# mikekatz04/Eryn

Measured on AMD Instinct MI355X. Metric: walker-steps/sec (ntemps x nwalkers x iters/s), Gaussian logL, higher is better.
Workload: dtype f64; 1 GPU; config 2: ntemps=16, nwalkers=4096, ndim=32 dense-covariance Gaussian, box prior +-50, StretchMove(a=2)+adaptive PT, Philox RNG; ntemps=16, nwalkers=4096, ndim=32, parallelism=single GPU

## Files before the change

### eryn_amd/csrc/hens_kernels.h

```cpp
#pragma once
#include <hip/hip_runtime.h>
#include <stdint.h>
#include <type_traits>

namespace hens {

constexpr int TILE = 64;
constexpr unsigned FLAG_NONFINITE_X = 1u;
constexpr unsigned FLAG_NAN_LOGL = 2u;

constexpr unsigned FLAG_PIPE_TIMEOUT = 4u;

enum { LIKE_DENSE = 0, LIKE_DIAG = 1, LIKE_ROSEN = 2, LIKE_HOST = 3 };
enum { MODE_STRETCH = 0, MODE_EVAL = 1, MODE_MH = 2 };

struct u4 { uint32_t x, y, z, w; };

__device__ __forceinline__ u4 philox4x32_10(u4 c, uint32_t k0, uint32_t k1) {
#pragma unroll
    for (int r = 0; r < 10; ++r) {
        const uint32_t hi0 = __umulhi(0xD2511F53u, c.x), lo0 = 0xD2511F53u * c.x;
        const uint32_t hi1 = __umulhi(0xCD9E8D57u, c.z), lo1 = 0xCD9E8D57u * c.z;
        c = u4{hi1 ^ c.y ^ k0, lo1, hi0 ^ c.w ^ k1, lo0};
        k0 += 0x9E3779B9u;
// ... 2188 lines not shown
            A.dbg_uacc[base + q] = sd.ua;
        }
    }
}

inline __global__ void k_plan_keys(const PlanArgs A, int nb) {
    const int g = blockIdx.x * blockDim.x + threadIdx.x;
    if (g >= nb * A.Tl) return;
    const int ib = g / A.Tl, job = g - ib * A.Tl;
    const uint32_t rung = (uint32_t)(A.rung_begin + job);
    const PrpKey K = prp_key(A.seed, A.iter0 + (uint64_t)ib, PURPOSE_PTPERM, rung);
    uint32_t* dst = A.keys + ((size_t)ib * A.T + rung) * 8;
#pragma unroll
    for (int r = 0; r < 8; ++r) dst[r] = K.k[r];
}

inline __global__ __launch_bounds__(256) void k_plan_draws(const PlanArgs A) {
    const int ib = blockIdx.y / A.Tl, job = blockIdx.y - ib * A.Tl;
    const uint32_t rung = (uint32_t)(A.rung_begin + job);
    const uint64_t it = A.iter0 + (uint64_t)ib;
    const int W = A.W, hb = A.cb >> 1, hb_shift = __ffs(hb) - 1, N0 = W >> 1;
    const int q = blockIdx.x * 256 + threadIdx.x;
    if (q >= W) return;
    const uint4* kp = reinterpret_cast<const uint4*>(A.keys + ((size_t)ib * A.T + rung) * 8);
    const uint4 ka = kp[0], kb = kp[1];
    const uint32_t key[8] = {ka.x, ka.y, ka.z, ka.w, kb.x, kb.y, kb.z, kb.w};
    const size_t base = ((size_t)ib * A.Tl + job) * W;
    const bool s0 = q < N0;
    const int p = s0 ? q : q - N0;
    const PlaceDraw pd = stretch_draws_at(A.seed, it, rung, q, key, W, A.idx_bits, hb_shift);
    const DrawRec rc = draw_values(pd.own, pd.cw, pd.uz, pd.ua, A.a, A.D);
    const int blk = p >> hb_shift, ml = p & (hb - 1);
    const size_t ri = ((size_t)ib * (W / A.cb) + blk) * TILE + (size_t)rung * hb + ml;
    if (A.rec1) {
        if (s0) {
            A.rec1[ri] = rc;
        } else {
            A.rec[ri] = rc;
            const PlaceDraw p1 = stretch_draws_at(A.seed, it, rung, pd.r, key, W, A.idx_bits, hb_shift);
            A.rec3[ri] = draw_values(p1.own, p1.cw, p1.uz, p1.ua, A.a, A.D);
        }
        return;
    }
    A.dr.own[base + q] = rc.own;
    if (s0 || !(A.rec && A.rec_only)) {
        A.dr.cw[base + q] = rc.cw;
        A.dr.zz[base + q] = rc.zz;
        A.dr.fac[base + q] = rc.fac;
        A.dr.lu[base + q] = rc.lu;
    }
    if (A.rec && !s0) A.rec[ri] = rc;
    if (A.dbg_uzz) {
        A.dbg_uzz[base + q] = pd.uz;
        A.dbg_uacc[base + q] = pd.ua;
    }
}

inline __global__ void k_pt_invert(const int64_t* __restrict__ iperm, int32_t* __restrict__ inv, int npairs, int W) {
    const int64_t n = (int64_t)npairs * W;
    for (int64_t i = blockIdx.x * (int64_t)blockDim.x + threadIdx.x; i < n; i += (int64_t)gridDim.x * blockDim.x) {
        const int j = (int)(i / W);
        inv[(size_t)j * W + iperm[i]] = (int32_t)(i - (int64_t)j * W);
    }
}

inline __global__ void k_pt_chain(const int64_t* __restrict__ iperm, const int64_t* __restrict__ i1perm,
                           const int32_t* __restrict__ inv, const double* __restrict__ u_swap,
                           int32_t* __restrict__ colslot, int32_t* __restrict__ colk,
                           double* __restrict__ colu, int T, int W) {
    const int c = blockIdx.x * blockDim.x + threadIdx.x;
    if (c >= W) return;
    int k = c;
    for (int j = 0; j < T - 1; ++j) {
        const int i = T - 1 - j;
        if (j == 0) colslot[(size_t)i * W + c] = (int32_t)iperm[k];
        const int b = (int)i1perm[(size_t)j * W + k];
        colslot[(size_t)(i - 1) * W + c] = b;
        colk[(size_t)j * W + c] = k;
        colu[(size_t)j * W + c] = u_swap[(size_t)j * W + k];
        if (j + 1 < T - 1) k = inv[(size_t)(j + 1) * W + b];
    }
}

struct PtArgs {
    const double* Lfull;
    const double* P;
    const int32_t* loc;
    double* Lnew;
    double* Pnew;
    int32_t* locnew;
    const WalkerRec* wrec;
    WalkerRec* wrecnew;
    const double* betas;
    const int32_t* colslot;
    const double* colu;
    uint8_t* selcol;
    int32_t* srcfull;
    uint32_t* swap_part;
    uint64_t iter;
    uint64_t seed;
    unsigned long long* trace;
    int32_t T, W, Tl, rung_begin, idx_bits;
    int32_t acc_rows;
};

constexpr int PT_COLS = 16;
constexpr int PT_THREADS = 256;
__host__ __device__ inline int pt_threads(int T) { const int ne = (T * 16 + 63) & ~63; return ne < 256 ? 256 : (ne > 1024 ? 1024 : ne); }

__host__ __device__ inline size_t pt_lds_layout(int T) { return (size_t)T * PT_COLS * (8 + 8 + 8 + 4 + 4) + (size_t)T * 8 + (size_t)PT_COLS * ((T + 31) / 32) * 4; }

template <bool PHILOX>
__global__ __launch_bounds__(1024) void k_pt_cascade(const PtArgs A) {
    extern __shared__ __attribute__((aligned(16))) char smem_raw[];
    const int T = A.T, W = A.W;
    const size_t NE = (size_t)T * PT_COLS;
    double* Lc = reinterpret_cast<double*>(smem_raw);
    double* lu = Lc + NE;
    double* Pc = lu + NE;
    double* sbeta = Pc + NE;
    int32_t* locc = reinterpret_cast<int32_t*>(sbeta + T);
    int32_t* scol = locc + NE;
    uint32_t* smask = reinterpret_cast<uint32_t*>(scol + NE);
    const int MW = (T + 31) / 32;
    const int tid = threadIdx.x;
    const int NTH = blockDim.x;
    const int c0 = blockIdx.x * PT_COLS;
    const uint64_t it = A.iter;
#define PT_TRACE(i) do { if (A.trace && tid == 0) A.trace[(size_t)blockIdx.x * 8 + (i)] = trace_stamp(); } while (0)
    PT_TRACE(0);

    for (int t = tid; t < T; t += NTH) sbeta[t] = A.betas[t];
    constexpr int PT_KEEP = 2;
    uint32_t acc_keep[PT_KEEP] = {0u, 0u};
    for (int e = tid, k = 0; e < (int)NE; e += NTH, ++k) {
        const int t = e / PT_COLS, cc = e - t * PT_COLS, c = c0 + cc;
        if (c < W) {
            const int slot = PHILOX ? pt_slot(A.seed, it, t, T, c, A.idx_bits, W) : A.colslot[(size_t)t * W + c];
            scol[e] = slot;
            const int tl = t - A.rung_begin;
            if (A.wrec) {
                const WalkerRec wr = A.wrec[(size_t)t * W + slot];
                Lc[e] = wr.L; Pc[e] = wr.P; locc[e] = wr.loc;
                if (k == 0) acc_keep[0] = wr.acc;
                if (k == 1) acc_keep[1] = wr.acc;
            } else {
                Lc[e] = A.Lfull[(size_t)t * W + slot];
                if (tl >= 0 && tl < A.Tl) {
                    Pc[e] = A.P[(size_t)tl * W + slot];
                    locc[e] = A.loc[(size_t)tl * W + slot];
                } else {
                    locc[e] = -1;
                }
            }
            if (t < T - 1) {
                const double u = PHILOX ? pt_uniform(A.seed, it, t, W, c) : A.colu[(size_t)t * W + c];
                lu[e] = log(u);
            }
        }
    }
    PT_TRACE(1);
    PT_TRACE(2);
    __syncthreads();
    PT_TRACE(3);

    auto walk = [&](auto tt) {
        constexpr int TT = decltype(tt)::value;
        const int Tn = TT ? TT : T;
        const int cc = tid;
        double cL = Lc[(size_t)(Tn - 1) * PT_COLS + cc];
        uint32_t m = 0;
#pragma unroll
        for (int i0 = Tn - 1; i0 >= 1; i0 -= 8) {
            double Lb[8], lv[8], db[8];
#pragma unroll
            for (int q = 0; q < 8; ++q) {
                const int i = (i0 - q >= 1) ? i0 - q : 1;
                Lb[q] = Lc[(size_t)(i - 1) * PT_COLS + cc];
                lv[q] = lu[(size_t)(Tn - 1 - i) * PT_COLS + cc];
                db[q] = sbeta[i - 1] - sbeta[i];
            }
#pragma unroll
            for (int q = 0; q < 8; ++q) {
                const int i = i0 - q;
                if (i >= 1) {
                    const double pacc = db[q] * (cL - Lb[q]);
                    const bool sw = pacc > lv[q];
                    m |= sw ? (1u << (i & 31)) : 0u;
                    cL = sw ? cL : Lb[q];
                    if ((i & 31) == 0 || i == 1) {
                        smask[cc * MW + (i >> 5)] = m;
                        m = 0;
                    }
                }
            }
        }
    };
    if (tid < PT_COLS && c0 + tid < W) {
        if (T == 8) walk(std::integral_constant<int, 8>{});
        else if (T == 16) walk(std::integral_constant<int, 16>{});
        else if (T == 32) walk(std::integral_constant<int, 32>{});
        else walk(std::integral_constant<int, 0>{});
    }
    PT_TRACE(4);
    __syncthreads();
    PT_TRACE(5);

    auto bit = [&](int cc, int i) -> bool { return (i >= 1 && i < T) && ((smask[cc * MW + (i >> 5)] >> (i & 31)) & 1u); };
    for (int e = tid, k = 0; e < (int)NE; e += NTH, ++k) {
        const int t = e / PT_COLS, cc = e - t * PT_COLS, c = c0 + cc;
        if (c >= W) continue;
        int st;
        bool sel_out;
        if (MW == 1) {
            const uint32_t mw = smask[cc];
            sel_out = (mw >> ((T - 1 - t) & 31)) & 1u;
            if ((mw >> t) & 1u) st = t - 1;
            else st = t + __builtin_ctz(~(mw >> 1 >> t));
        } else {
            sel_out = bit(cc, T - 1 - t);
            if (bit(cc, t)) {
                st = t - 1;
            } else {
                st = t;
                while (bit(cc, st + 1)) ++st;
            }
        }
        if (t < T - 1 && A.selcol) A.selcol[(size_t)t * W + c] = sel_out ? 1 : 0;
        const int se = st * PT_COLS + cc;
        const int dslot = scol[e];
        if (A.srcfull) A.srcfull[(size_t)t * W + dslot] = st * W + scol[se];
        const int tl = t - A.rung_begin;
        if (tl < 0 || tl >= A.Tl) continue;
        const size_t di = (size_t)tl * W + dslot;
        if (A.wrecnew) {
            const uint32_t acc_own = (k < PT_KEEP && A.rung_begin == 0) ? (k == 0 ? acc_keep[0] : acc_keep[1]) : A.wrec[di].acc;
            A.wrecnew[di] = make_wrec(Lc[se], Pc[se], locc[se], acc_own);
            A.locnew[di] = locc[se];
            continue;
        }
        A.Lnew[di] = Lc[se];
        A.locnew[di] = locc[se];
        if (locc[se] >= 0) A.Pnew[di] = Pc[se];
    }
    for (int i = 1 + tid; i < T; i += NTH) {
        unsigned n = 0;
        for (int cc = 0; cc < PT_COLS && c0 + cc < W; ++cc) n += bit(cc, i) ? 1u : 0u;
        if (A.acc_rows) { if (n) atomicAdd(&A.swap_part[(size_t)(blockIdx.x & (A.acc_rows - 1)) * (T - 1) + (i - 1)], n); }
        else A.swap_part[(size_t)blockIdx.x * (T - 1) + (i - 1)] = n;
    }
    PT_TRACE(6);
#undef PT_TRACE
}

constexpr int SWAP_ACC_ROWS_MAX = 64;
__host__ __device__ inline int acc_row_groups(int T) {
    int p2 = 1;
    while (p2 < T - 1) p2 <<= 1;
    const int g = p2 >= 64 ? 1 : 64 / p2;
    return g > SWAP_ACC_ROWS_MAX / 8 ? SWAP_ACC_ROWS_MAX / 8 : g;
}

struct FusedArgs {
    double* pool;
    const WalkerRec* wrec;
    WalkerRec* wrecnew;
    const int32_t* loc;
    int32_t* locnew;
    const double* betas;
    const uint32_t* keys;
    const uint32_t* keys_next;
    uint32_t* accepted;
    uint32_t* swap_acc;
    const double* lo; const double* hi; const double* mu; const double* prec; const double* prec_sym;
    const double* period;
    unsigned* flags;
    unsigned long long* trace;
    double logp_in, fill, rosen_a, rosen_b;
    double a;
    uint64_t iter, seed;
    int32_t T, W, idx_bits, cb, cb_shift, ndim_active;
    int32_t acc_rows;
    int32_t norel;
    int32_t Tl, rung_begin;
    int32_t cbl, cbl_shift;
    int64_t guest_delta;
    int32_t* ghome;
    char* box; char* box_hot; char* box_cold;
    const double* pool_cold;
    unsigned long long* stats;
    long long budget;
    uint32_t sweep;
    int32_t par, nranks, rank;
    int32_t sys_rows;
    int32_t no_move;
};

__host__ __device__ constexpr size_t fused_lds_base(int D, int NW, bool pipe = false) {
    return ((size_t)TILE * (D + 2) + (size_t)NW * TILE + 5 * TILE + 3 * 2 * TILE + 64 + (pipe ? 2 * TILE : 0)) * 8 +
           (2 * 2 * TILE + 5 * TILE + 64 + (pipe ? 3 * TILE : 0)) * 4;
}
__host__ __device__ inline size_t fused_lds_bytes(int D, int NW, int like, bool pipe = false) { return fused_lds_base(D, NW, pipe) + mf_lds_extra(D, like); }

template <int DT, int LIKE, int NW, bool PER = false, bool SHORT = false, bool PIPE = false, bool COL = false>
__global__ __launch_bounds__(NW * 64) void k_split1_pt(const FusedArgs A) {
    static_assert(DT == 8 || DT == 16 || DT == 32 || DT == 64 || DT == 128, "power-of-two row width");
    static_assert(!(PIPE && SHORT), "pipeline ranks: full tiles");
    static_assert(!(COL && (PER || SHORT)), "column-ordered records: full tiles");
    extern __shared__ __attribute__((aligned(16))) char smem_raw[];
    constexpr bool CEN = like_centred(LIKE, DT);
    constexpr int D = DT, RS = DT + 2, NT = NW * 64, LPR = DT / 2, RPP = NT / LPR, NPASS = (TILE + RPP - 1) / RPP;
    constexpr int NE = 2 * TILE;
    constexpr int NEX = PIPE ? NE + TILE : NE;
    static_assert(NT >= 2 * NE, "one thread per slot + one per cascade uniform");
    constexpr bool WIDE = NT >= 2 * NE + 64;
    double* qtile = reinterpret_cast<double*>(smem_raw);
    double* s_part = qtile + TILE * RS;
    double* s_zz = s_part + NW * TILE;
    double* s_fac = s_zz + TILE;
    double* s_lu = s_fac + TILE;
    double* s_Lold = s_lu + TILE;
    double* s_Pold = s_Lold + TILE;
    int2* s_own = reinterpret_cast<int2*>(s_Lold);
    double* Lc = s_Pold + TILE;
    double* Pc = Lc + NEX;
    double* lupt = Pc + NEX;
    double* sbeta = lupt + NE;
    int32_t* locc = reinterpret_cast<int32_t*>(sbeta + 64);
    int32_t* scol = locc + NEX;
    int32_t* s_rs = scol + NE;
    int32_t* s_rc = s_rs + TILE;
    int32_t* s_dst = s_rc + TILE;
    int32_t* s_flag = s_dst + TILE;
    int32_t* s_el = s_flag + TILE;
    uint32_t* smask = reinterpret_cast<uint32_t*>(s_el + TILE);
    int32_t* s_src = reinterpret_cast<int32_t*>(smask + 64);
    int32_t* s_yrow = s_src + TILE;
    double* s_mu = reinterpret_cast<double*>(smem_raw + fused_lds_base(DT, NW, PIPE));

    const int tid = threadIdx.x;
    const int lane = tid & 63;
    const int wv = __builtin_amdgcn_readfirstlane(tid >> 6);
    if constexpr (like_mf<DT, LIKE, NW>()) {
        if (tid >= NW * 64 - DT / 2) *reinterpret_cast<double2*>(s_mu + 2 * (tid - (NW * 64 - DT / 2))) = *reinterpret_cast<const double2*>(A.mu + 2 * (tid - (NW * 64 - DT / 2)));
    }
    MfRegs mfr = like_prefetch<DT == 32 ? DT : 0, LIKE, NW>(lane, wv, A.prec_sym);
    const int TG = A.T;
    const int T = PIPE ? A.Tl : A.T;
    const int W = A.W, CB = PIPE ? A.cbl : A.cb, CS = PIPE ? A.cbl_shift : A.cb_shift;
    const int R0 = PIPE ? A.rung_begin : 0;
    const bool has_top = PIPE && R0 + T < TG, has_bot = PIPE && R0 > 0;
    const int TE = T + (has_top ? 1 : 0);
    const int c0 = blockIdx.x * CB;
    const int MW = (TE + 31) >> 5;
    const int NEr = SHORT ? (T << CS) : 2 * TILE, NM = SHORT ? (NEr >> 1) : TILE;
#define FUSED_TRACE(i) do { if (A.trace && tid == 0) A.trace[(size_t)blockIdx.x * 8 + (i)] = trace_stamp(); } while (0)
    FUSED_TRACE(0);
#ifdef HENS_DEV_BUILD
    if (HENS_CUT_F == 9) return;
#endif
#ifdef HENS_DEV_BUILD
    if (HENS_CUT_F == 8) {
        const long long t0 = wall_clock64();
        while (wall_clock64() - t0 < 600) __builtin_amdgcn_s_sleep(4);
        return;
    }
#endif

    WalkerRec wr_n{};
    bool stays = false;
    int slot_n = 0;
    int32_t home_n = 0;
    const int HS = A.cb_shift - 1, HB = 1 << HS;
    const int HW = CB >> 1;
    const bool nomove = PIPE && A.no_move != 0;
    constexpr int CWW = WIDE ? 5 : 2, FLW = WIDE ? 6 : 3;
    auto mover_of = [&](int t, int cc) -> int {
        if (PIPE) return (t << (CS - 1)) + ((cc >> (HS + 1)) << HS) + (cc & (HB - 1));
        return (t << (CS - 1)) + cc - HB;
    };
    if (wv == 0) s_flag[lane] = 0;
    if (tid < NEr) {
        const int e = tid, t = e >> CS, cc = e & (CB - 1), c = c0 + cc;
        if (COL) {
            wr_n = A.wrec[(size_t)t * W + c];
        } else {
            const uint4* kp = reinterpret_cast<const uint4*>(A.keys) + (size_t)(R0 + t) * 2;
            const uint4 ka = kp[0], kb = kp[1];
            const uint32_t key[8] = {ka.x, ka.y, ka.z, ka.w, kb.x, kb.y, kb.z, kb.w};
            slot_n = (int)prp((uint32_t)c, key, A.idx_bits, (uint32_t)W);
            wr_n = A.wrec[(size_t)t * W + slot_n];
        }
        stays = PIPE ? (nomove || ((cc >> HS) & 1) == 0) : cc < HB;
        if (!stays) {
            const int m = mover_of(t, cc);
            s_rs[m] = wr_n.loc;
            if (PIPE) home_n = A.ghome[wr_n.loc < 0 ? ~wr_n.loc : 0];
            else s_dst[m] = t * W + slot_n;
        }
        if (!COL) scol[e] = slot_n;
        if (!WIDE && e < TE) sbeta[e] = A.betas[R0 + e];
    }
    if (tid >= NE && tid < 2 * NE) {
        const int e = tid - NE, t = e >> CS, c = c0 + (e & (CB - 1));
        if (t < TE - 1) lupt[e] = log(pt_uniform(A.seed, A.iter, PIPE ? TG - R0 - TE + t : t, W, c));
    }
    constexpr bool ONEDRAW = COL && WIDE;
    if (COL && WIDE && !ONEDRAW && wv == 3 && lane < NM) {
        const int m = lane, t = m >> (CS - 1), q = (W >> 1) + blockIdx.x * HW + (m & (HW - 1));
        s_lu[m] = log(stretch_draw(A.seed, A.iter, (uint32_t)(R0 + t) * (uint32_t)W + (uint32_t)q).ua);
    }
    if (COL && (NW >= 8 ? (wv == 4 || wv == 7) : wv < 2)) {
        const int e = (NW >= 8 ? (wv == 4 ? 0 : 64) : wv * 64) + lane, t = e >> CS, c = c0 + (e & (CB - 1));
        const uint32_t slot = (uint32_t)A.wrec[(size_t)t * W + c].slot;
        const uint4* kn = reinterpret_cast<const uint4*>(A.keys_next) + (size_t)(R0 + t) * 2;
        const uint4 na = kn[0], nb = kn[1];
        const uint32_t keyn[8] = {na.x, na.y, na.z, na.w, nb.x, nb.y, nb.z, nb.w};
        scol[e] = (int)prp_inv(slot, keyn, A.idx_bits, (uint32_t)W);
    }
    if (WIDE && wv == (ONEDRAW ? FLW : 4)) {
        if (lane < TE) sbeta[lane] = A.betas[R0 + lane];
    }
    if (ONEDRAW && wv == CWW && lane < NM && !nomove) {
        const int m = lane, t = m >> (CS - 1), q = (W >> 1) + blockIdx.x * HW + (m & (HW - 1));
        const StretchDraw sd = stretch_draw(A.seed, A.iter, (uint32_t)(R0 + t) * (uint32_t)W + (uint32_t)q);
        const int cw = place_column(0, stretch_index(sd.r22, W >> 1), HS);
        const int32_t rcv = A.loc[t * W + cw];
        const double z = draw_zz(sd.uz, A.a);
        s_zz[m] = z;
        s_fac[m] = ((double)A.ndim_active - 1.0) * log(z);
        s_rc[m] = rcv;
    }
    if (ONEDRAW && wv == FLW && lane < NM && !nomove) {
        const int m = lane, t = m >> (CS - 1), q = (W >> 1) + blockIdx.x * HW + (m & (HW - 1));
        s_lu[m] = log(stretch_draw(A.seed, A.iter, (uint32_t)(R0 + t) * (uint32_t)W + (uint32_t)q).ua);
    }
    if (!ONEDRAW && (wv == CWW || wv == FLW) && lane < NM && !nomove) {
        const int m = lane, t = m >> (CS - 1), q = (W >> 1) + blockIdx.x * HW + (m & (HW - 1));
        const StretchDraw sd = stretch_draw(A.seed, A.iter, (uint32_t)(R0 + t) * (uint32_t)W + (uint32_t)q);
        if (wv == CWW) {
            int cw;
            if (COL) {
                cw = place_column(0, stretch_index(sd.r22, W >> 1), HS);
            } else {
                const uint4* kp = reinterpret_cast<const uint4*>(A.keys) + (size_t)(R0 + t) * 2;
                const uint4 ka = kp[0], kb = kp[1];
                const uint32_t key[8] = {ka.x, ka.y, ka.z, ka.w, kb.x, kb.y, kb.z, kb.w};
                cw = (int)prp((uint32_t)place_column(0, stretch_index(sd.r22, W >> 1), HS), key, A.idx_bits, (uint32_t)W);
            }
            s_rc[m] = A.loc[t * W + cw];
        }
        if (wv == FLW || CWW == FLW) {
            if (COL && WIDE) {
                const double z = draw_zz(sd.uz, A.a);
                s_zz[m] = z;
                s_fac[m] = ((double)A.ndim_active - 1.0) * log(z);
            } else {
                const DrawRec dv = draw_values(0, 0, sd.uz, sd.ua, A.a, A.ndim_active);
                s_zz[m] = dv.zz; s_fac[m] = dv.fac; s_lu[m] = dv.lu;
            }
        }
    }
#ifdef HENS_TRACE_WAVES
    if (A.trace && lane == 0 && wv >= 1 && wv < 8) A.trace[(size_t)blockIdx.x * 8 + wv] = trace_stamp();
    if (A.trace && tid == 0) { lds_barrier(); return; }
#endif
    FUSED_TRACE(1);
    lds_barrier();
    FUSED_TRACE(2);
#ifdef HENS_DEV_BUILD
    if (HENS_CUT_F == 1) return;
#endif

    const int jl = tid & (LPR - 1);
    const int rsub = tid / LPR;
    const double* __restrict__ pool_r = A.pool;
    double2 sreg[NPASS], creg[NPASS];
    bool rv[NPASS];
    int rs_i[NPASS], rc_i[NPASS];
#pragma unroll
    for (int p = 0; p < NPASS; ++p) {
        const int rr = p * RPP + rsub < TILE ? p * RPP + rsub : 0;
        rs_i[p] = s_rs[rr];
        rc_i[p] = s_rc[rr];
    }
#pragma unroll
    for (int p = 0; p < NPASS; ++p) {
        const int r = p * RPP + rsub;
        rv[p] = r < NM && !nomove;
        sreg[p] = double2{0.0, 0.0};
        creg[p] = double2{0.0, 0.0};
        if (rv[p]) {
            sreg[p] = *reinterpret_cast<const double2*>(pool_r + (PIPE ? row_off(rs_i[p], D, A.guest_delta) : (int64_t)rs_i[p] * D) + jl * 2);
            creg[p] = *reinterpret_cast<const double2*>(pool_r + (PIPE ? row_off(rc_i[p], D, A.guest_delta) : (int64_t)rc_i[p] * D) + jl * 2);
        }
    }
    const double2 lov = *reinterpret_cast<const double2*>(A.lo + jl * 2);
    const double2 hiv = *reinterpret_cast<const double2*>(A.hi + jl * 2);
    double2 muv = double2{0.0, 0.0};
    if (CEN) muv = *reinterpret_cast<const double2*>(A.mu + jl * 2);
    double2 qkeep[NPASS];
    if (tid < NEr && stays) {
        Lc[tid] = wr_n.L; Pc[tid] = wr_n.P; locc[tid] = wr_n.loc;
    }
#pragma unroll
    for (int p = 0; p < NPASS; ++p) {
        const int r = p * RPP + rsub;
        bool ok = true, finite = true;
        if (rv[p]) {
            const double zz = s_zz[r];
            double2 qv;
            qv.x = creg[p].x - (creg[p].x - sreg[p].x) * zz;
            qv.y = creg[p].y - (creg[p].y - sreg[p].y) * zz;
            if (PER) {
                const double2 pv = *reinterpret_cast<const double2*>(A.period + jl * 2);
                qv.x = periodic_wrap(creg[p].x - periodic_diff(sreg[p].x, creg[p].x, pv.x) * zz, pv.x);
                qv.y = periodic_wrap(creg[p].y - periodic_diff(sreg[p].y, creg[p].y, pv.y) * zz, pv.y);
            }
            ok = (qv.x >= lov.x) && (qv.x <= hiv.x) && (qv.y >= lov.y) && (qv.y <= hiv.y);
            finite = (fabs(qv.x) < INFINITY) && (fabs(qv.y) < INFINITY);
            if (CEN) qkeep[p] = qv;
            *reinterpret_cast<double2*>(qtile + r * RS + jl * 2) = double2{qv.x - muv.x, qv.y - muv.y};
        }
        const unsigned long long bad = __ballot(!ok);
        const unsigned long long nonfin = __ballot(!finite);
        const int gshift = lane & ~(LPR - 1);
        const unsigned long long gmask = (LPR == 64) ? ~0ull : (((1ull << (LPR & 63)) - 1ull) << gshift);
        if (jl == 0 && rv[p]) {
            if ((bad & gmask) == 0ull) atomicOr(&s_flag[r], 1);
            if ((nonfin & gmask) != 0ull) atomicOr(A.flags, FLAG_NONFINITE_X);
        }
    }
    if constexpr (DT != 32) mfr = like_prefetch<DT, LIKE, NW>(lane, wv, A.prec_sym);
    FUSED_TRACE(3);
    lds_barrier();
#ifdef HENS_DEV_BUILD
    if (HENS_CUT_F == 2) return;
#endif

    if (!nomove) {
        const bool inbox = (s_flag[lane] & 1) != 0;
        like_partials<DT, LIKE, NW, CEN>(qtile, s_part, lane, wv, inbox, like_mf<DT, LIKE, NW>() ? s_mu : A.mu, A.prec, A.prec_sym, A.rosen_a, A.rosen_b, mfr);
    }
    FUSED_TRACE(4);
    lds_barrier();
#ifdef HENS_DEV_BUILD
    if (HENS_CUT_F == 3) return;
#endif

    if (tid < NEr && !stays) {
        const int e = tid, t = e >> CS, m = mover_of(t, e & (CB - 1));
        const bool inbox = (s_flag[m] & 1) != 0;
        double acc = 0.0;
#pragma unroll
        for (int w2 = 0; w2 < like_nparts<DT, LIKE, NW>(); ++w2) acc += s_part[w2 * TILE + m];
        double logl = inbox ? -0.5 * acc : A.fill;
        if (logl != logl) {
            logl = -1e300;
            atomicOr(A.flags, FLAG_NAN_LOGL);
        }
        const double logp = inbox ? A.logp_in : -INFINITY;
        const double beta = sbeta[t];
        const double Lold = wr_n.L, Pold = wr_n.P;
        double lt = logl * beta;
        if (lt != lt) lt = -INFINITY;
        const double logP = lt + logp;
        double lo_ = Lold * beta;
        if (lo_ != lo_) lo_ = -INFINITY;
        const double prevP = lo_ + Pold;
        const double lnpdiff = s_fac[m] + logP - prevP;
        const bool keep = lnpdiff > s_lu[m];
        const double newP = (fabs(logp) == INFINITY) ? 0.0 : logp;
        Lc[e] = keep ? logl : Lold;
        Pc[e] = keep ? newP : Pold;
        if (PIPE) {
            const bool guest = wr_n.loc < 0;
            const int32_t row = guest ? home_n : wr_n.loc;
            locc[e] = row;
            s_dst[m] = row;
            if (guest) s_flag[m] |= 8;
        } else {
            locc[e] = wr_n.loc;
        }
        if (keep) {
            wr_n.acc += 1u;
            s_flag[m] |= 2;
        }
    }
    if (tid < NEr) s_own[tid] = int2{(int)wr_n.acc, wr_n.slot};
    FUSED_TRACE(5);
    lds_barrier();
#ifdef HENS_DEV_BUILD
    if (HENS_CUT_F == 4) return;
#endif

    auto walk = [&](auto tt) {
        constexpr int TT = decltype(tt)::value;
        const int Tn = TT ? TT : TE;
        const int cc = lane;
        double cL = Lc[((Tn - 1) << CS) + cc];
        uint32_t m = 0;
#pragma unroll
        for (int i0 = Tn - 1; i0 >= 1; i0 -= 8) {
            double Lb[8], lv[8], db[8];
#pragma unroll
            for (int q = 0; q < 8; ++q) {
                const int i = (i0 - q >= 1) ? i0 - q : 1;
                Lb[q] = Lc[((i - 1) << CS) + cc];
                lv[q] = lupt[((Tn - 1 - i) << CS) + cc];
                db[q] = sbeta[i - 1] - sbeta[i];
            }
#pragma unroll
            for (int q = 0; q < 8; ++q) {
                const int i = i0 - q;
                if (i >= 1) {
                    const double pacc = db[q] * (cL - Lb[q]);
                    const bool sw = pacc > lv[q];
                    m |= sw ? (1u << (i & 31)) : 0u;
                    cL = sw ? cL : Lb[q];
                    if ((i & 31) == 0 || i == 1) {
                        smask[cc * MW + (i >> 5)] = m;
                        m = 0;
                    }
                }
            }
        }
    };
    const bool walking = wv == (NW > 1 ? 1 : 0);
    auto store_accepted = [&]() {
        if constexpr (PIPE) {
            double2 val[NPASS];
            double* dstp[NPASS];
            bool on[NPASS];
#pragma unroll
            for (int p = 0; p < NPASS; ++p) {
                const int r = p * RPP + rsub;
                on[p] = false;
                val[p] = double2{0.0, 0.0};
                dstp[p] = A.pool;
                if (!rv[p]) continue;
                const int fl = s_flag[r];
                const double2 ql = CEN ? qkeep[p] : *reinterpret_cast<const double2*>(qtile + r * RS + jl * 2);
                const bool acc = (fl & 2) != 0;
                double2 o = sreg[p];
                if constexpr (DT == 128) {
                    o = double2{0.0, 0.0};
                    if (!acc && (fl & 8)) o = *reinterpret_cast<const double2*>(A.pool + row_off(s_rs[r], D, A.guest_delta) + jl * 2);
                }
                val[p].x = acc ? ql.x : o.x;
                val[p].y = acc ? ql.y : o.y;
                on[p] = (fl & (2 | 8)) != 0;
                dstp[p] = A.pool + (size_t)s_dst[r] * D + jl * 2;
            }
            if (A.sys_rows) {
#pragma unroll
                for (int p = 0; p < NPASS; ++p) if (on[p]) store_row16_sys(dstp[p], val[p]);
            } else {
#pragma unroll
                for (int p = 0; p < NPASS; ++p) if (on[p]) store_row16(dstp[p], val[p]);
            }
        } else {
#pragma unroll
            for (int p = 0; p < NPASS; ++p) {
                const int r = p * RPP + rsub;
                if (!rv[p]) continue;
                if ((s_flag[r] & 2) == 0) continue;
                store_row16(A.pool + (size_t)s_rs[r] * D + jl * 2,
                            CEN ? qkeep[p] : *reinterpret_cast<const double2*>(qtile + r * RS + jl * 2));
            }
        }
    };
    if (PIPE) {
        store_accepted();
        char* const box_l = late_kernarg<char*>(offsetof(FusedArgs, box));
        char* const box_hot_l = late_kernarg<char*>(offsetof(FusedArgs, box_hot));
        const int32_t par_l = late_kernarg<int32_t>(offsetof(FusedArgs, par));
        const uint32_t sweep_l = late_kernarg<uint32_t>(offsetof(FusedArgs, sweep));
        const long long budget_l = late_kernarg<long long>(offsetof(FusedArgs, budget));
        unsigned long long* const stats_l = late_kernarg<unsigned long long*>(offsetof(FusedArgs, stats));
        const PipeBox me = pipe_box(box_l, TG, W, D);
        if (has_top) {
            if (tid >= ((T - 1) << CS) && tid < (T << CS)) {
                const PipeBox hot = pipe_box(box_hot_l, TG, W, D);
                const int slot = COL ? c0 + (tid & (CB - 1)) : scol[tid];
                sys_store(hot.lp_dn + (size_t)(par_l * 2) * W + slot, Lc[tid]);
                sys_store(hot.lp_dn + (size_t)(par_l * 2 + 1) * W + slot, Pc[tid]);
                __hip_atomic_store(hot.ldn_loc + (size_t)par_l * W + slot, locc[tid], __ATOMIC_RELAXED, __HIP_MEMORY_SCOPE_SYSTEM);
            }
            asm volatile("s_waitcnt vmcnt(0)" ::: "memory");
            __syncthreads();
            if (tid == 0) pipe_raise(pipe_box(box_hot_l, TG, W, D).blk_ldn + blockIdx.x, sweep_l + 1);
            if (walking) {
                if (lane == 0) pipe_spin(me.blk_lup + blockIdx.x, sweep_l + 1, budget_l, A.flags, stats_l ? stats_l + 4 : nullptr);
                if (lane < CB) {
                    const int c = c0 + lane, et = (T << CS) + lane;
                    Lc[et] = sys_load(me.lp_up + (size_t)(par_l * 2) * W + c);
                    Pc[et] = sys_load(me.lp_up + (size_t)(par_l * 2 + 1) * W + c);
                    locc[et] = pipe_guest_loc(par_l, 0, W, c);
                }
            }
        }
        if (walking && lane < CB) {
            if (TE == 9) walk(std::integral_constant<int, 9>{});
            else if (TE == 8) walk(std::integral_constant<int, 8>{});
            else if (TE == 16) walk(std::integral_constant<int, 16>{});
            else if (TE == 17) walk(std::integral_constant<int, 17>{});
            else if (TE == 4) walk(std::integral_constant<int, 4>{});
            else if (TE == 5) walk(std::integral_constant<int, 5>{});
            else if (TE == 1) smask[lane * MW] = 0;
            else walk(std::integral_constant<int, 0>{});
        }
    } else {
        if (!walking) store_accepted();
        if (walking && lane < CB) {
            if (T == 16) walk(std::integral_constant<int, 16>{});
            else if (T == 8) walk(std::integral_constant<int, 8>{});
            else if (T == 32) walk(std::integral_constant<int, 32>{});
            else walk(std::integral_constant<int, 0>{});
        }
    }
    lds_barrier();
    FUSED_TRACE(6);
#ifdef HENS_DEV_BUILD
    if (HENS_CUT_F == 5) return;
#endif

    auto bit = [&](int cc, int i) -> bool { return (i >= 1 && i < TE) && ((smask[cc * MW + (i >> 5)] >> (i & 31)) & 1u); };
    int se_n = 0;
    auto settles = [&](const int e) -> int {
        const int t = e >> CS, cc = e & (CB - 1);
        int st;
        if (MW == 1) {
            const uint32_t mw = smask[cc];
            if ((mw >> t) & 1u) st = t - 1;
            else st = t + __builtin_ctz(~(mw >> 1 >> t));
        } else if (bit(cc, t)) {
            st = t - 1;
        } else {
            st = t;
            while (bit(cc, st + 1)) ++st;
        }
        return (st << CS) + cc;
    };
    const bool paired = PIPE || late_kernarg<int32_t>(offsetof(FusedArgs, norel)) != 0;
    if (PIPE && tid < NEr) {
        se_n = settles(tid);
        if (has_top && (se_n >> CS) == T)
            A.ghome[(size_t)(late_kernarg<int32_t>(offsetof(FusedArgs, par)) * 2) * W + c0 + (tid & (CB - 1))] = locc[((T - 1) << CS) + (tid & (CB - 1))];
    }
    if (paired ? tid < 2 * NEr : tid < NEr) {
        const int e = paired ? tid >> 1 : tid, t = e >> CS;
        const int se = settles(e);
        const size_t di = (size_t)t * W + scol[e];
        WalkerRec* const wrecnew_l = late_kernarg<WalkerRec*>(offsetof(FusedArgs, wrecnew));
        int32_t* const locnew_l = late_kernarg<int32_t*>(offsetof(FusedArgs, locnew));
        if (paired) {
            const int h = tid & 1;
            const int2 own = s_own[e];
            const double2 v = h == 0 ? double2{Lc[se], Pc[se]} : double2{__hiloint2double(own.x, locc[se]), __hiloint2double(0, own.y)};
            store_row16(reinterpret_cast<double*>(&wrecnew_l[di]) + 2 * h, v);
            if (h == 1) wt_store(&locnew_l[di], locc[se]);
        } else {
            wrecnew_l[di] = make_wrec(Lc[se], Pc[se], locc[se], wr_n.acc, wr_n.slot);
            locnew_l[di] = locc[se];
        }
    }
    for (int i = 1 + tid; i < TE; i += NT) {
        unsigned n = 0;
        for (int cc = 0; cc < CB; ++cc) n += bit(cc, i) ? 1u : 0u;
        if (n) {
            uint32_t* const acc_l = late_kernarg<uint32_t*>(offsetof(FusedArgs, swap_acc));
            const int32_t rows_l = late_kernarg<int32_t>(offsetof(FusedArgs, acc_rows));
            atomicAdd(&acc_l[(size_t)(blockIdx.x & (rows_l - 1)) * (TE - 1) + (i - 1)], n);
        }
    }
    if (!PIPE && walking) store_accepted();

    if constexpr (PIPE) {
        char* const box_l = late_kernarg<char*>(offsetof(FusedArgs, box));
        char* const box_cold_l = late_kernarg<char*>(offsetof(FusedArgs, box_cold));
        const double* const pool_cold_l = late_kernarg<const double*>(offsetof(FusedArgs, pool_cold));
        const int32_t par_l = late_kernarg<int32_t>(offsetof(FusedArgs, par));
        const uint32_t sweep_l = late_kernarg<uint32_t>(offsetof(FusedArgs, sweep));
        const long long budget_l = late_kernarg<long long>(offsetof(FusedArgs, budget));
        unsigned long long* const stats_l = late_kernarg<unsigned long long*>(offsetof(FusedArgs, stats));
        const PipeBox me = pipe_box(box_l, TG, W, D);
        if (has_bot) {
            const PipeBox cold = pipe_box(box_cold_l, TG, W, D);
            if (tid < CB) {
                sys_store(cold.lp_up + (size_t)(par_l * 2) * W + c0 + tid, Lc[se_n]);
                sys_store(cold.lp_up + (size_t)(par_l * 2 + 1) * W + c0 + tid, Pc[se_n]);
            }
            asm volatile("s_waitcnt vmcnt(0)" ::: "memory");
            __syncthreads();
            if (tid == 0) pipe_raise(cold.blk_lup + blockIdx.x, sweep_l + 1);
            if (tid == 0) pipe_spin(me.blk_ldn + blockIdx.x, sweep_l + 1, budget_l, A.flags, stats_l ? stats_l + 6 : nullptr);
            if (tid == 64 && has_top) pipe_spin(me.blk_rows + blockIdx.x, sweep_l + 1, budget_l, A.flags, stats_l ? stats_l + 8 : nullptr);
            __syncthreads();
            if (tid < CB) {
                const int cc = tid, c = c0 + cc, g = R0;
                int slot_below = c;
                if (!COL) {
                    const uint4* kp = reinterpret_cast<const uint4*>(A.keys) + (size_t)(g - 1) * 2;
                    const uint4 ka = kp[0], kb = kp[1];
                    const uint32_t key[8] = {ka.x, ka.y, ka.z, ka.w, kb.x, kb.y, kb.z, kb.w};
                    slot_below = (int)prp((uint32_t)c, key, A.idx_bits, (uint32_t)W);
                }
                const double La = Lc[se_n];
                const double Lb = sys_load(me.lp_dn + (size_t)(par_l * 2) * W + slot_below);
                const double db = A.betas[g - 1] - A.betas[g];
                int32_t src = PIPE_NOSEL, yrow = 0;
                if (db * (La - Lb) > log(pt_uniform(A.seed, A.iter, TG - 1 - g, W, c))) {
                    src = locc[se_n];
                    yrow = __hip_atomic_load(me.ldn_loc + (size_t)par_l * W + slot_below, __ATOMIC_RELAXED, __HIP_MEMORY_SCOPE_SYSTEM);
                    const double Pb = sys_load(me.lp_dn + (size_t)(par_l * 2 + 1) * W + slot_below);
                    const int32_t gl = pipe_guest_loc(par_l, 1, W, c);
                    const size_t di = (size_t)scol[tid];
                    late_kernarg<WalkerRec*>(offsetof(FusedArgs, wrecnew))[di] = make_wrec(Lb, Pb, gl, wr_n.acc, wr_n.slot);
                    late_kernarg<int32_t*>(offsetof(FusedArgs, locnew))[di] = gl;
                    A.ghome[(size_t)(par_l * 2 + 1) * W + c] = src >= 0 ? src : locc[((T - 1) << CS) + cc];
                }
                s_src[cc] = src;
                s_yrow[cc] = yrow;
            }
            __syncthreads();
            {
                double* dst = cold.guest + (size_t)(par_l * 2) * W * D;
                double* mine = me.guest + (size_t)(par_l * 2 + 1) * W * D;
                for (int base = 0; base < CB * D; base += 4 * NT) {
                    double push[4], pull[4];
                    bool on[4];
#pragma unroll
                    for (int q = 0; q < 4; ++q) {
                        const int idx = base + q * NT + tid;
                        on[q] = false;
                        if (idx < CB * D) {
                            const int col = idx / D, d = idx - col * D;
// ... 627 lines not shown
```

Measured before the change: 4.107 billion walker-steps/s.

## Defer per-wave setup roles past first barrier to shorten the pre-barrier critical path

For column-ordered wide kernels with D<=64, several side tasks are moved after the first LDS barrier: the PT uniform logs, the inverse permutation of next-iteration keys, the log(z) factor, the acceptance uniform draw and the beta stores. Before the barrier, the global loads are only issued and held in registers, so the slowest wave reaches the barrier sooner. The deferred work then overlaps with the pool row loads and the proposal construction, which run before the second barrier. This adds register pressure, forces explicit waitcnt instructions, and requires an 8-wave block layout.

```diff
diff --git a/eryn_amd/csrc/hens_kernels.h b/eryn_amd/csrc/hens_kernels.h
--- a/eryn_amd/csrc/hens_kernels.h
+++ b/eryn_amd/csrc/hens_kernels.h
@@ -2514,6 +2514,15 @@
 }
 __host__ __device__ inline size_t fused_lds_bytes(int D, int NW, int like, bool pipe = false) { return fused_lds_base(D, NW, pipe) + mf_lds_extra(D, like); }
 
+__host__ __device__ constexpr bool late_roles_ok(int D, int like) {
+#ifdef HENS_HEAD_ROLES
+    return false;
+#else
+    (void)like;
+    return D <= 64;
+#endif
+}
+
 template <int DT, int LIKE, int NW, bool PER = false, bool SHORT = false, bool PIPE = false, bool COL = false>
 __global__ __launch_bounds__(NW * 64) void k_split1_pt(const FusedArgs A) {
     static_assert(DT == 8 || DT == 16 || DT == 32 || DT == 64 || DT == 128, "power-of-two row width");
@@ -2613,10 +2622,15 @@
         if (!COL) scol[e] = slot_n;
         if (!WIDE && e < TE) sbeta[e] = A.betas[R0 + e];
     }
-    if (tid >= NE && tid < 2 * NE) {
+    constexpr bool LATE = COL && WIDE && !PIPE && late_roles_ok(DT, LIKE);
+    uint32_t late_slot = 0;
+    uint4 late_ka{}, late_kb{};
+    double late_z = 1.0, late_beta = 0.0;
+    auto lupt_role = [&]() {
         const int e = tid - NE, t = e >> CS, c = c0 + (e & (CB - 1));
         if (t < TE - 1) lupt[e] = log(pt_uniform(A.seed, A.iter, PIPE ? TG - R0 - TE + t : t, W, c));
-    }
+    };
+    if (!LATE && tid >= NE && tid < 2 * NE) lupt_role();
     constexpr bool ONEDRAW = COL && WIDE;
     if (COL && WIDE && !ONEDRAW && wv == 3 && lane < NM) {
         const int m = lane, t = m >> (CS - 1), q = (W >> 1) + blockIdx.x * HW + (m & (HW - 1));
@@ -2627,11 +2641,21 @@
         const uint32_t slot = (uint32_t)A.wrec[(size_t)t * W + c].slot;
         const uint4* kn = reinterpret_cast<const uint4*>(A.keys_next) + (size_t)(R0 + t) * 2;
         const uint4 na = kn[0], nb = kn[1];
-        const uint32_t keyn[8] = {na.x, na.y, na.z, na.w, nb.x, nb.y, nb.z, nb.w};
-        scol[e] = (int)prp_inv(slot, keyn, A.idx_bits, (uint32_t)W);
+        if (LATE) {
+            late_slot = slot; late_ka = na; late_kb = nb;
+            __builtin_amdgcn_s_waitcnt(0x0F70);
+        } else {
+            const uint32_t keyn[8] = {na.x, na.y, na.z, na.w, nb.x, nb.y, nb.z, nb.w};
+            scol[e] = (int)prp_inv(slot, keyn, A.idx_bits, (uint32_t)W);
+        }
     }
     if (WIDE && wv == (ONEDRAW ? FLW : 4)) {
-        if (lane < TE) sbeta[lane] = A.betas[R0 + lane];
+        if (LATE) {
+            if (lane < TE) late_beta = A.betas[R0 + lane];
+            __builtin_amdgcn_s_waitcnt(0x0F70);
+        } else {
+            if (lane < TE) sbeta[lane] = A.betas[R0 + lane];
+        }
     }
     if (ONEDRAW && wv == CWW && lane < NM && !nomove) {
         const int m = lane, t = m >> (CS - 1), q = (W >> 1) + blockIdx.x * HW + (m & (HW - 1));
@@ -2640,13 +2664,29 @@
         const int32_t rcv = A.loc[t * W + cw];
         const double z = draw_zz(sd.uz, A.a);
         s_zz[m] = z;
-        s_fac[m] = ((double)A.ndim_active - 1.0) * log(z);
+        if (LATE) late_z = z;
+        else s_fac[m] = ((double)A.ndim_active - 1.0) * log(z);
         s_rc[m] = rcv;
     }
-    if (ONEDRAW && wv == FLW && lane < NM && !nomove) {
+    auto lu_role = [&]() {
         const int m = lane, t = m >> (CS - 1), q = (W >> 1) + blockIdx.x * HW + (m & (HW - 1));
         s_lu[m] = log(stretch_draw(A.seed, A.iter, (uint32_t)(R0 + t) * (uint32_t)W + (uint32_t)q).ua);
-    }
+    };
+    if (ONEDRAW && !LATE && wv == FLW && lane < NM && !nomove) lu_role();
+    auto late_roles = [&]() {
+        if (wv == 2 || wv == 3) {
+            lupt_role();
+        } else if (wv == 4 || wv == 7) {
+            const int e = (wv == 4 ? 0 : 64) + lane;
+            const uint32_t keyn[8] = {late_ka.x, late_ka.y, late_ka.z, late_ka.w, late_kb.x, late_kb.y, late_kb.z, late_kb.w};
+            scol[e] = (int)prp_inv(late_slot, keyn, A.idx_bits, (uint32_t)W);
+        } else if (wv == CWW) {
+            if (lane < NM) s_fac[lane] = ((double)A.ndim_active - 1.0) * log(late_z);
+        } else if (wv == FLW) {
+            if (lane < NM) lu_role();
+            if (lane < TE) sbeta[lane] = late_beta;
+        }
+    };
     if (!ONEDRAW && (wv == CWW || wv == FLW) && lane < NM && !nomove) {
         const int m = lane, t = m >> (CS - 1), q = (W >> 1) + blockIdx.x * HW + (m & (HW - 1));
         const StretchDraw sd = stretch_draw(A.seed, A.iter, (uint32_t)(R0 + t) * (uint32_t)W + (uint32_t)q);
@@ -2673,13 +2713,19 @@
             }
         }
     }
+    static_assert(!LATE || NW == 8, "late roles: the 8-wave role assignment");
 #ifdef HENS_TRACE_WAVES
-    if (A.trace && lane == 0 && wv >= 1 && wv < 8) A.trace[(size_t)blockIdx.x * 8 + wv] = trace_stamp();
-    if (A.trace && tid == 0) { lds_barrier(); return; }
-#endif
+#define HENS_TRACE_WAVES_AT (HENS_TRACE_WAVES + 0 == 2 ? 2 : 1)
+    if (HENS_TRACE_WAVES_AT == 1 && A.trace && lane == 0 && wv >= 1 && wv < 8) A.trace[(size_t)blockIdx.x * 8 + wv] = trace_stamp();
+    if (HENS_TRACE_WAVES_AT == 1 && A.trace && tid == 0) { lds_barrier(); return; }
+    if (HENS_TRACE_WAVES_AT == 1) FUSED_TRACE(1);
+    lds_barrier();
+    if (HENS_TRACE_WAVES_AT == 1) FUSED_TRACE(2);
+#else
     FUSED_TRACE(1);
     lds_barrier();
     FUSED_TRACE(2);
+#endif
 #ifdef HENS_DEV_BUILD
     if (HENS_CUT_F == 1) return;
 #endif
@@ -2715,6 +2761,7 @@
     if (tid < NEr && stays) {
         Lc[tid] = wr_n.L; Pc[tid] = wr_n.P; locc[tid] = wr_n.loc;
     }
+    if constexpr (LATE) late_roles();
 #pragma unroll
     for (int p = 0; p < NPASS; ++p) {
         const int r = p * RPP + rsub;
@@ -2744,7 +2791,12 @@
         }
     }
     if constexpr (DT != 32) mfr = like_prefetch<DT, LIKE, NW>(lane, wv, A.prec_sym);
+#ifdef HENS_TRACE_WAVES
+    if (HENS_TRACE_WAVES_AT == 2 && A.trace && lane == 0 && wv >= 1 && wv < 8) A.trace[(size_t)blockIdx.x * 8 + wv] = trace_stamp();
+    if (HENS_TRACE_WAVES_AT == 2 && A.trace && tid == 0) { lds_barrier(); return; }
+#else
     FUSED_TRACE(3);
+#endif
     lds_barrier();
 #ifdef HENS_DEV_BUILD
     if (HENS_CUT_F == 2) return;
```

Measured after the change: 4.064 billion walker-steps/s. 1.0% lower.
